# DaehwanKimLab/hisat-genotype

Measured on AMD Instinct MI355X. Metric: typed reads/sec at HLA-A (~7k alleles, 2x150bp), higher is better.
Workload: dtype u64 bitsets, f64 EM

## Files before the change

hisat-genotype_amd/capi.py:

```python
import ctypes as C
import threading
import os

import numpy as np

HERE = os.path.dirname(os.path.abspath(__file__))
LIB_PATH = os.path.join(HERE, "csrc", "libhgx.so")
LAB_PATH = os.path.join(HERE, "csrc", "lab", "libhgx_lab.so")

VAR_INSERTION, VAR_SINGLE, VAR_DELETION = 0, 1, 2
BASE_KIND = {"hla": 0, "codis": 1, "genome": 2}


class HgxError(RuntimeError):
    def __init__(self, code, msg):
        super().__init__("libhgx error %d: %s" % (code, msg))
        self.code = code


class HgxKeyError(HgxError, KeyError):
    """The reference raises KeyError at this point (EM quirk Q6)."""


class Piece(C.Structure):
    _fields_ = [("mask_off", C.c_uint32), ("lo_word", C.c_uint16), ("n_words", C.c_uint16)]


PIECE_DTYPE = np.dtype([("mask_off", np.uint32), ("lo_word", np.uint16), ("n_words", np.uint16)])


class LocusDesc(C.Structure):
    _fields_ = [("base_kind", C.c_int32), ("backbone_len", C.c_int32), ("backbone", C.c_char_p),
                ("n_vars", C.c_int32), ("var_pos", C.c_void_p), ("var_type", C.c_void_p), ("var_len", C.c_void_p),
                ("var_base", C.c_void_p), ("var_linked", C.c_void_p), ("var_name_pool", C.c_char_p),
                ("var_ins_pool", C.c_char_p), ("n_alleles", C.c_int32), ("link_off", C.c_void_p),
                ("link_allele", C.c_void_p), ("n_link_order", C.c_int32), ("link_order", C.c_void_p),
                ("n_exons", C.c_int32), ("exons", C.c_void_p), ("allele_len", C.c_void_p), ("name_rank", C.c_void_p)]


class ParseOpts(C.Structure):
    _fields_ = [("num_editdist", C.c_int32), ("error_correction", C.c_int32), ("allow_discordant", C.c_int32),
                ("simulation", C.c_int32), ("base_locus", C.c_int32), ("keep_trace", C.c_int32),
                ("codis_choose_pairs", C.c_int32), ("n_threads", C.c_int32),
                ("pileup_exchange", C.c_void_p), ("pileup_ctx", C.c_void_p),
                ("interdist_exchange", C.c_void_p), ("interdist_ctx", C.c_void_p),
                ("pileup_exchange_dev", C.c_void_p), ("pileup_dev_ctx", C.c_void_p)]


PILEUP_EXCHANGE = C.CFUNCTYPE(C.c_int, C.c_void_p, C.POINTER(C.c_uint32), C.c_int64)
PILEUP_EXCHANGE_DEV = C.CFUNCTYPE(C.c_int, C.c_void_p, C.c_void_p, C.c_int64, C.c_void_p)
INTERDIST_EXCHANGE = C.CFUNCTYPE(C.c_int, C.c_void_p, C.POINTER(C.c_int64), C.c_int64)


SYMBOLS = [
    "hgx_last_error", "hgx_version", "hgx_device_count", "hgx_set_device", "hgx_dev_alloc", "hgx_dev_free",
    "hgx_memcpy_h2d", "hgx_memcpy_h2d_async", "hgx_memcpy_d2h", "hgx_memset", "hgx_stream_sync", "hgx_stream_create", "hgx_stream_create_prio", "hgx_stream_destroy", "hgx_pool_trim", "hgx_event_create", "hgx_event_destroy",
    "hgx_event_record", "hgx_stream_wait_event", "hgx_event_elapsed_ms", "hgx_a_pad", "hgx_index_create",
    "hgx_index_destroy", "hgx_index_dims", "hgx_index_device_bits", "hgx_piece_compat", "hgx_pair_classes",
    "hgx_score_pairs", "hgx_level_classes", "hgx_group_pairs", "hgx_groups_dims", "hgx_groups_destroy",
    "hgx_level_classes_grouped", "hgx_classes_set_allele_rank", "hgx_dedup_classes", "hgx_classes_destroy", "hgx_classes_dims", "hgx_classes_device",
    "hgx_classes_to_host", "hgx_classes_from_host", "hgx_allele_counts", "hgx_allele_counts_on", "hgx_first_classes", "hgx_em", "hgx_em_ordered", "hgx_em_masked", "hgx_em_set_backend", "hgx_test_switch_set", "hgx_debug_matvec", "hgx_em_set_timing", "hgx_em_get_timing", "hgx_locus_create",
    "hgx_locus_destroy", "hgx_locus_dims", "hgx_locus_tables", "hgx_index_from_locus",
    "hgx_locus_alternatives_text", "hgx_batch_destroy", "hgx_batch_dims", "hgx_batch_arrays",
    "hgx_batch_from_haplotypes", "hgx_parse_sam", "hgx_read_alignments", "hgx_free_text", "hgx_parse_alignment_file", "hgx_batch_trace_text", "hgx_batch_pileup",
    "hgx_dbatch_create", "hgx_dbatch_destroy", "hgx_dbatch_dims", "hgx_gate_create", "hgx_gate_destroy", "hgx_type_dbatch",
    "hgx_type_batch", "hgx_type_file", "hgx_typing_destroy", "hgx_typing_dims", "hgx_typing_counts", "hgx_typing_em",
    "hgx_typing_gene_prob", "hgx_typing_classes", "hgx_write_bam", "hgx_em_last_exact", "hgx_index_device_block", "hgx_index_create_device", "hgx_type_classes", "hgx_pair_classes_dedup",
    "hgx_bgzf_inflate", "hgx_bgzf_inflate_verdicts", "hgx_bgzf_scan_compare", "hgx_many_create", "hgx_many_create_files", "hgx_many_create_sams", "hgx_many_tasks", "hgx_many_destroy", "hgx_many_dims", "hgx_type_many", "hgx_type_many_loci", "hgx_em_set_fast", "hgx_em_last_order", "hgx_typing_top", "hgx_emx_set_timing", "hgx_emx_get_timing",
    "hgx_index_broadcast", "hgx_allreduce_sum_u32", "hgx_allreduce_sum_i64", "hgx_classes_allgather",
    "hgx_classes_pack_rows", "hgx_classes_merge_gathered", "hgx_rccl_stats",
    "hgx_keyset_create", "hgx_keyset_dims", "hgx_keyset_fill", "hgx_keyset_destroy",
    "hgx_many_from_dbatch", "hgx_alignment_open", "hgx_alignment_dims", "hgx_alignment_parse_dev", "hgx_alignment_close", "hgx_stream_sets_info", "hgx_stream_create_placed", "hgx_stream_probe_matrix", "hgx_stream_probe_pair", "hgx_stream_probe_chain", "hgx_stream_sets_streams",
    "hgx_parse_sam_dev", "hgx_parse_alignment_file_dev", "hgx_front_last", "hgx_front_last_parts", "hgx_dbatch_to_host",
    "hgx_emx_cluster_stats", "hgx_em_tie_reruns",
    "hgx_linear_locus_create", "hgx_linear_locus_destroy", "hgx_linear_type_sam", "hgx_linear_type_file", "hgx_linear_dims",
    "hgx_linear_counts", "hgx_linear_classes", "hgx_linear_extra_names", "hgx_linear_destroy",
    "hgx_linear_input_open", "hgx_linear_input_dims", "hgx_linear_type_input", "hgx_linear_input_close",
    "hgx_alignment_set_open", "hgx_alignment_set_dims", "hgx_alignment_set_info", "hgx_alignment_set_route", "hgx_alignment_set_routed",
    "hgx_alignment_set_close", "hgx_many_create_set",
    "hgx_bam_index_build", "hgx_bam_index_last", "hgx_bam_splice",
    "hgx_extract_open", "hgx_extract_feed", "hgx_extract_feed_bam", "hgx_extract_file", "hgx_extract_take", "hgx_extract_stats", "hgx_extract_close",
    "hgx_align_index_create", "hgx_align_index_free", "hgx_align_reads", "hgx_align_last", "hgx_align_last_states",
    "hgx_align_last_pairs", "hgx_align_last_clip", "hgx_align_reads_x", "hgx_align_last_gap",
]

_lib = None


def lib():
    global _lib
    if _lib is None:
        if not os.path.exists(LIB_PATH):
            raise ImportError("libhgx.so is not built: run `python -c 'import __graft_entry__ as g; g.build()'` "
                              "(hipcc --offload-arch=gfx950); there is no CPU fallback")
        _lib = C.CDLL(LIB_PATH)
        _lib.hgx_last_error.restype = C.c_char_p
        _lib.hgx_a_pad.restype = C.c_int32
    return _lib


def use_lab():
    global LIB_PATH
    if _lib is not None:
        raise RuntimeError("libhgx.so is already loaded in this process")
    LIB_PATH = LAB_PATH


def check(rc):
    if rc != 0:
        msg = lib().hgx_last_error().decode(errors="replace")
        if rc == -4:
            raise HgxKeyError(rc, msg)
        raise HgxError(rc, msg)


def ptr(a):
    if a is None:
        return None
    if hasattr(a, "ptr") and not hasattr(a, "ctypes"):
        return C.c_void_p(a.ptr)
    return a.ctypes.data_as(C.c_void_p)


def a_pad(n_alleles):
    return int(lib().hgx_a_pad(C.c_int32(n_alleles)))


def device_count():
    n = C.c_int(0)
    check(lib().hgx_device_count(C.byref(n)))
    return n.value


_current_device = 0
_streams = {}


def set_device(dev):
    global _current_device
    check(lib().hgx_set_device(C.c_int(dev)))
    _current_device = dev


def current_device():
    return _current_device


_slot = threading.local()


def set_stream_slot(k):
    _slot.k = ("slot", k)


def get_stream(i):
    key = (_current_device, getattr(_slot, "k", threading.get_ident()), i)
    if key not in _streams:
        p = C.c_void_p()
        fn = lib().hgx_stream_create_placed if i == 2 else lib().hgx_stream_create_prio
        check(fn(C.byref(p), C.c_int(1 if i == 0 else 0)))
        _streams[key] = p
    return _streams[key]


class DevArray:

    def __init__(self, shape, dtype):
        self.shape = tuple(int(x) for x in (shape if isinstance(shape, (tuple, list)) else (shape,)))
        self.dtype = np.dtype(dtype)
        self.nbytes = int(np.prod(self.shape, dtype=np.int64)) * self.dtype.itemsize
        p = C.c_void_p()
        check(lib().hgx_dev_alloc(C.byref(p), C.c_size_t(self.nbytes)))
        self.ptr = p.value

    @staticmethod
    def from_host(arr, stream=None, sync=True):
        arr = np.ascontiguousarray(arr)
        d = DevArray(arr.shape, arr.dtype)
        if arr.nbytes:
            fn = lib().hgx_memcpy_h2d if sync else lib().hgx_memcpy_h2d_async
            check(fn(C.c_void_p(d.ptr), ptr(arr), C.c_size_t(arr.nbytes), stream))
        return d

    def to_host(self, stream=None):
        out = np.empty(self.shape, dtype=self.dtype)
        if self.nbytes:
            check(lib().hgx_memcpy_d2h(ptr(out), C.c_void_p(self.ptr), C.c_size_t(self.nbytes), stream))
        return out

    def zero(self, stream=None):
        check(lib().hgx_memset(C.c_void_p(self.ptr), 0, C.c_size_t(self.nbytes), stream))

    def free(self):
        if self.ptr:
            lib().hgx_dev_free(C.c_void_p(self.ptr))
            self.ptr = None

    def __del__(self):
        try:
            self.free()
        except Exception:
            pass


def sync(stream=None):
    check(lib().hgx_stream_sync(stream))


class Event:

    def __init__(self):
# ... 21 lines not shown
```

hisat-genotype_amd/csrc/hgx_device.hip:

```cpp
#include <hip/hip_runtime.h>

#include <algorithm>
#include <cstdarg>
#include <cstdio>
#include <cstring>
#include <vector>

#include <map>
#include <mutex>
#include <unordered_map>

#include "hgx_common.hpp"

static thread_local char g_err[512] = "";

extern "C" void hgx_set_error(const char *fmt, ...) {
    va_list ap;
    va_start(ap, fmt);
    vsnprintf(g_err, sizeof(g_err), fmt, ap);
    va_end(ap);
}
extern "C" const char *hgx_last_error(void) { return g_err; }
extern "C" int hgx_version(void) { return 100; }


extern "C" int hgx_device_count(int *n) { HIPCHK(hipGetDeviceCount(n)); return HGX_OK; }
namespace {
struct Staging {
    char *buf = nullptr;
    size_t cap = 0, used = 0;
    struct Pending { void *dst; const char *src; size_t n; };
    std::vector<Pending> pending;
    std::vector<hipStream_t> streams;
    void note(hipStream_t st) {
        for (auto s : streams) if (s == st) return;
        streams.push_back(st);
    }
    static std::mutex &mu() { static std::mutex m; return m; }
    static std::vector<char *> &free_list() { static std::vector<char *> v; return v; }
    ~Staging() {
        if (buf) { std::lock_guard<std::mutex> g(mu()); free_list().push_back(buf); }
    }
    char *take(size_t n) {
        const size_t need = (n + 63) & ~(size_t)63;
        if (!buf) {
            cap = 1u << 20;
            {
                std::lock_guard<std::mutex> g(mu());
                if (!free_list().empty()) { buf = free_list().back(); free_list().pop_back(); }
            }
            if (!buf && hipHostMalloc((void **)&buf, cap) != hipSuccess) { buf = nullptr; cap = 0; return nullptr; }
        }
        if (used + need > cap) return nullptr;
        char *r = buf + used;
        used += need;
        return r;
    }
};
thread_local Staging g_stage;
constexpr size_t STAGE_MAX = 256u << 10;
}

int hgx_d2h(void *dst, const void *src, size_t n, hipStream_t st) {
    char *s = n <= STAGE_MAX ? g_stage.take(n) : nullptr;
    if (!s) { HIPCHK(hipMemcpyAsync(dst, src, n, hipMemcpyDeviceToHost, st)); return HGX_OK; }
    HIPCHK(hipMemcpyAsync(s, src, n, hipMemcpyDeviceToHost, st));
    g_stage.pending.push_back({dst, s, n});
    g_stage.note(st);
    return HGX_OK;
}
int hgx_h2d(void *dst, const void *src, size_t n, hipStream_t st) {
    char *s = n <= STAGE_MAX ? g_stage.take(n) : nullptr;
    if (!s) { HIPCHK(hipMemcpyAsync(dst, src, n, hipMemcpyHostToDevice, st)); return HGX_OK; }
    memcpy(s, src, n);
    HIPCHK(hipMemcpyAsync(dst, s, n, hipMemcpyHostToDevice, st));
    g_stage.note(st);
    return HGX_OK;
}
int hgx_sync(hipStream_t st) {
    HIPCHK(hipStreamSynchronize(st));
    for (auto s2 : g_stage.streams) if (s2 != st) HIPCHK(hipStreamSynchronize(s2));
    g_stage.streams.clear();
    for (auto &p : g_stage.pending) memcpy(p.dst, p.src, p.n);
    g_stage.pending.clear();
    g_stage.used = 0;
    return HGX_OK;
}

extern "C" int hgx_set_device(int dev) { HIPCHK(hipSetDevice(dev)); return HGX_OK; }
void *hgx_pool_alloc(size_t bytes);
void hgx_pool_free(void *p);
extern "C" int hgx_dev_alloc(void **p, size_t bytes) {
    ARGCHK(p != nullptr);
    if (bytes <= (16u << 20)) {
        *p = hgx_pool_alloc(bytes);
        if (!*p) { hgx_set_error("device allocation of %zu bytes failed", bytes); return HGX_ENOMEM; }
        return HGX_OK;
    }
    HIPCHK(hipMalloc(p, bytes));
    return HGX_OK;
}
extern "C" int hgx_dev_free(void *p) { hgx_pool_free(p); return HGX_OK; }
extern "C" int hgx_memcpy_h2d(void *d, const void *s, size_t n, void *st) {
    int rc = hgx_h2d(d, s, n, (hipStream_t)st);
    return rc ? rc : hgx_sync((hipStream_t)st);
}
extern "C" int hgx_memcpy_h2d_async(void *d, const void *s, size_t n, void *st) {
    if (n > STAGE_MAX) return hgx_memcpy_h2d(d, s, n, st);
    return hgx_h2d(d, s, n, (hipStream_t)st);
}
extern "C" int hgx_memcpy_d2h(void *d, const void *s, size_t n, void *st) {
    int rc = hgx_d2h(d, s, n, (hipStream_t)st);
    return rc ? rc : hgx_sync((hipStream_t)st);
}
extern "C" int hgx_memset(void *d, int v, size_t n, void *st) {
    HIPCHK(hipMemsetAsync(d, v, n, (hipStream_t)st));
    return HGX_OK;
}
extern "C" int hgx_stream_sync(void *st) { return hgx_sync((hipStream_t)st); }
extern "C" int hgx_stream_create(void **st) {
    ARGCHK(st != nullptr);
    hipStream_t s;
    HIPCHK(hipStreamCreateWithFlags(&s, hipStreamNonBlocking));
    *st = (void *)s;
    return HGX_OK;
}
extern "C" int hgx_stream_create_prio(void **st, int high_priority) {
    ARGCHK(st != nullptr);
    int least = 0, greatest = 0;
    HIPCHK(hipDeviceGetStreamPriorityRange(&least, &greatest));
    hipStream_t s;
    HIPCHK(hipStreamCreateWithPriority(&s, hipStreamNonBlocking, high_priority ? greatest : least));
    *st = (void *)s;
    return HGX_OK;
}
bool hgx_ss_forget_stream(void *stream);
extern "C" int hgx_stream_destroy(void *st) {
    if (st && !hgx_ss_forget_stream(st)) HIPCHK(hipStreamDestroy((hipStream_t)st));
    return HGX_OK;
}
extern "C" int hgx_event_create(void **ev) {
    ARGCHK(ev != nullptr);
    hipEvent_t e;
    HIPCHK(hipEventCreate(&e));
    *ev = (void *)e;
    return HGX_OK;
}
extern "C" int hgx_event_destroy(void *ev) { if (ev) HIPCHK(hipEventDestroy((hipEvent_t)ev)); return HGX_OK; }
extern "C" int hgx_event_record(void *ev, void *st) { HIPCHK(hipEventRecord((hipEvent_t)ev, (hipStream_t)st)); return HGX_OK; }
extern "C" int hgx_stream_wait_event(void *st, void *ev) { HIPCHK(hipStreamWaitEvent((hipStream_t)st, (hipEvent_t)ev, 0)); return HGX_OK; }
extern "C" int hgx_event_elapsed_ms(void *a, void *b, float *ms) {
    ARGCHK(a && b && ms);
    HIPCHK(hipEventSynchronize((hipEvent_t)b));
    HIPCHK(hipEventElapsedTime(ms, (hipEvent_t)a, (hipEvent_t)b));
    return HGX_OK;
}


namespace {
struct Pool {
    std::mutex mu;
    std::multimap<std::pair<int, size_t>, void *> free_blocks;
    std::unordered_map<void *, std::pair<int, size_t>> size_of;
};
int cur_device() { int d = 0; (void)hipGetDevice(&d); return d; }
Pool &pool() { static Pool p; return p; }
size_t round_size(size_t n) {
    size_t r = 256;
    while (r < n) r <<= 1;
    if (r > (1u << 20)) {
        const size_t step = r >> 4;
        r = (n + step - 1) / step * step;
    }
    return r;
}
}

void *hgx_pool_alloc(size_t bytes) {
    Pool &P = pool();
    const size_t sz = round_size(bytes ? bytes : 8);
    const int dev = cur_device();
    {
        std::lock_guard<std::mutex> g(P.mu);
        auto it = P.free_blocks.find({dev, sz});
        if (it != P.free_blocks.end()) {
            void *p = it->second;
            P.free_blocks.erase(it);
            return p;
        }
    }
    void *p = nullptr;
    if (hipMalloc(&p, sz) != hipSuccess) {
        {
            std::lock_guard<std::mutex> g(P.mu);
            for (auto it = P.free_blocks.begin(); it != P.free_blocks.end();) {
                if (it->first.first == dev) { P.size_of.erase(it->second); (void)hipFree(it->second); it = P.free_blocks.erase(it); }
                else ++it;
            }
        }
        if (hipMalloc(&p, sz) != hipSuccess) return nullptr;
    }
    std::lock_guard<std::mutex> g(P.mu);
    P.size_of[p] = {dev, sz};
    return p;
}
void hgx_pool_free(void *p) {
    if (!p) return;
    Pool &P = pool();
    std::lock_guard<std::mutex> g(P.mu);
    auto it = P.size_of.find(p);
    if (it == P.size_of.end()) { (void)hipFree(p); return; }
    P.free_blocks.emplace(it->second, p);
}
void hgx_host_pool_trim();
extern "C" int hgx_pool_trim(void) {
    hgx_host_pool_trim();
    Pool &P = pool();
    std::lock_guard<std::mutex> g(P.mu);
    for (auto &kv : P.free_blocks) { P.size_of.erase(kv.second); (void)hipFree(kv.second); }
    P.free_blocks.clear();
    return HGX_OK;
}


extern "C" int32_t hgx_a_pad(int32_t n) { return (n + 511) / 512 * 512; }

static int index_alloc(hgx_index **out, int32_t n_alleles, int32_t n_vars) {
    ARGCHK(out && n_alleles > 0 && n_vars >= 0);
    ARGCHK(n_vars <= 65535 * 32);
    hgx_index *ix = new hgx_index();
    ix->n_alleles = n_alleles;
    ix->a_pad = hgx_a_pad(n_alleles);
    ix->n_vars = n_vars;
    ix->n_words = std::max(1, (n_vars + 31) / 32);
    ix->w64 = ix->a_pad / 64;
    const size_t nb = (size_t)ix->n_words * ix->a_pad * sizeof(uint32_t);
    void *block = nullptr;
    if (hipMalloc(&block, nb + 2 * (size_t)ix->w64 * 8) != hipSuccess) {
        delete ix;
        hgx_set_error("device allocation of the locus index failed");
        return HGX_ENOMEM;
    }
    ix->d_bits = (uint32_t *)block;
    ix->d_exon_mask = (uint64_t *)((char *)block + nb);
    ix->d_gene_mask = ix->d_exon_mask + ix->w64;
    *out = ix;
    return HGX_OK;
}
extern "C" int hgx_index_create(hgx_index **out, int32_t n_alleles, int32_t n_vars, const uint32_t *bits,
                                const uint64_t *exon_mask, const uint64_t *gene_mask) {
    ARGCHK(out && bits && exon_mask && gene_mask);
    *out = nullptr;
    hgx_index *ix = nullptr;
    { int rc_ = index_alloc(&ix, n_alleles, n_vars); if (rc_) return rc_; }
    const size_t nb = (size_t)ix->n_words * ix->a_pad * sizeof(uint32_t);
    if (hipMemcpy(ix->d_bits, bits, nb, hipMemcpyHostToDevice) != hipSuccess ||
        hipMemcpy(ix->d_exon_mask, exon_mask, ix->w64 * 8, hipMemcpyHostToDevice) != hipSuccess ||
        hipMemcpy(ix->d_gene_mask, gene_mask, ix->w64 * 8, hipMemcpyHostToDevice) != hipSuccess) {
        (void)hipFree(ix->d_bits);
        delete ix;
        hgx_set_error("upload of the locus index failed");
        return HGX_EHIP;
    }
    *out = ix;
    return HGX_OK;
}
extern "C" int hgx_index_create_device(hgx_index **out, int32_t n_alleles, int32_t n_vars) {
    ARGCHK(out);
    *out = nullptr;
    return index_alloc(out, n_alleles, n_vars);
}
extern "C" int hgx_index_destroy(hgx_index *ix) {
    if (!ix) return HGX_OK;
    (void)hipFree(ix->d_bits);
    hgx_pool_free(ix->d_pid); hgx_pool_free(ix->d_vals); hgx_pool_free(ix->d_nval);
    delete ix->pat_mu;
    delete ix;
    return HGX_OK;
}
extern "C" int hgx_index_dims(const hgx_index *ix, int32_t *na, int32_t *ap, int32_t *nv, int32_t *nw) {
    ARGCHK(ix);
    if (na) *na = ix->n_alleles;
    if (ap) *ap = ix->a_pad;
    if (nv) *nv = ix->n_vars;
    if (nw) *nw = ix->n_words;
    return HGX_OK;
}
extern "C" int hgx_index_device_bits(const hgx_index *ix, void **p, size_t *bytes) {
    ARGCHK(ix && p && bytes);
    *p = ix->d_bits;
    *bytes = (size_t)ix->n_words * ix->a_pad * sizeof(uint32_t);
// ... 341 lines not shown
        for (int s = 0; s < kw; ++s) {
            const int w = lane + 64 * s;
            const bool live = w < w64;
            uint64_t plane[NP];
#pragma unroll
            for (int k = 0; k < NP; ++k) plane[k] = 0;
            for (int r = r0; r < r1; ++r) {
                const uint32_t ref = (uint32_t)__builtin_amdgcn_readfirstlane(refs[r]);
                if ((ref >> 31) != level) continue;
                uint64_t carry = live ? compat[(size_t)(ref & 0x7fffffffu) * w64 + w] : 0ull;
#pragma unroll
                for (int k = 0; k < NP; ++k) {
                    const uint64_t t = plane[k] & carry;
                    plane[k] ^= carry;
                    carry = t;
                }
            }
            uint64_t cand = live ? mask[w] : 0ull;
            if (pass == 0) {
                uint32_t v = 0;
#pragma unroll
                for (int k = NP - 1; k >= 0; --k) {
                    const uint64_t t = cand & plane[k];
                    if (__any(t != 0)) { cand = t; v |= 1u << k; }
                }
                gmax = max(gmax, v);
            } else {
#pragma unroll
                for (int k = 0; k < NP; ++k) cand &= ((gmax >> k) & 1u) ? plane[k] : ~plane[k];
                if (live) {
#ifdef HGX_LAB
                    if (fa) __hip_atomic_store((unsigned long long *)&out_row[w], (unsigned long long)cand, __ATOMIC_RELAXED, __HIP_MEMORY_SCOPE_AGENT);
                    else
#endif
                    if (out_row) out_row[w] = cand;
                    h += word_hash(cand, w);
                    nz = nz || cand != 0;
                }
            }
        }
#ifdef HGX_LAB
    if (fa) {
        h = wave_sum_u64(h);
        const uint64_t key = finish_hash(h, __any(nz));
        if (key == HGX_EMPTY_KEY) { if (lane == 0) fa->slot_of[pair] = 0xFFFFFFFFu; return; }
        asm volatile("s_waitcnt vmcnt(0)" ::: "memory");
        int won;
        const uint32_t slot = fused_find_slot(*fa, key, lane, won);
        if (lane == 0) fa->slot_of[pair] = slot;
        if (won) { if (lane == 0) __hip_atomic_store(&fa->rep[slot], (uint32_t)pair, __ATOMIC_RELAXED, __HIP_MEMORY_SCOPE_AGENT); return; }
        const uint32_t r = fused_wait_rep(*fa, slot, lane);
        bool diff = false;
        for (int w = lane; w < w64; w += 64)
            diff = diff || __hip_atomic_load((unsigned long long *)&fa->rows[(size_t)r * w64 + w], __ATOMIC_RELAXED, __HIP_MEMORY_SCOPE_AGENT) !=
                               __hip_atomic_load((unsigned long long *)&out_row[w], __ATOMIC_RELAXED, __HIP_MEMORY_SCOPE_AGENT);
        if (__any(diff) && lane == 0) atomicOr(fa->bad, 1);
        return;
    }
#endif
    if (out_hash) {
        h = wave_sum_u64(h);
        const bool any_nz = __any(nz);
        if (lane == 0) *out_hash = finish_hash(h, any_nz);
    }
}

template <int KW, bool SEL>
__global__ __launch_bounds__(256) void k_pair_classes(const uint64_t *__restrict__ compat, int w64,
                                                      const int32_t *__restrict__ pair_off, const uint32_t *__restrict__ refs,
                                                      const int64_t *__restrict__ sel,
                                                      int n_pairs, const uint64_t *__restrict__ exon_mask,
                                                      const uint64_t *__restrict__ gene_mask, uint64_t *__restrict__ exon_bits,
                                                      uint64_t *__restrict__ gene_bits, uint64_t *__restrict__ exon_hash,
                                                      uint64_t *__restrict__ gene_hash) {
    const int lane = threadIdx.x & 63;
    const long out = ((long)blockIdx.x * blockDim.x + threadIdx.x) >> 6;
    if (out >= n_pairs) return;
    const long pair = SEL ? (long)sel[out] : out;
    const int r0 = __builtin_amdgcn_readfirstlane(pair_off[pair]);
    const int r1 = __builtin_amdgcn_readfirstlane(pair_off[pair + 1]);
    const int n_refs = r1 - r0;
#define HGX_LEVELS(NP_)                                                                                                          \
    do {                                                                                                                         \
        if (exon_bits || exon_hash)                                                                                              \
            class_for_level<KW, NP_>(compat, w64, refs, r0, r1, 0u, exon_mask, exon_bits ? exon_bits + (size_t)out * w64 : nullptr, \
                                     exon_hash ? exon_hash + out : nullptr, lane);                                              \
        if (gene_bits || gene_hash)                                                                                              \
            class_for_level<KW, NP_>(compat, w64, refs, r0, r1, 1u, gene_mask, gene_bits ? gene_bits + (size_t)out * w64 : nullptr, \
                                     gene_hash ? gene_hash + out : nullptr, lane);                                              \
    } while (0)
    if (n_refs <= 3) HGX_LEVELS(2);
    else if (n_refs <= 15) HGX_LEVELS(4);
    else if (n_refs <= 255) HGX_LEVELS(8);
    else {
        if (exon_bits || exon_hash)
            class_for_level_wide(compat, w64, refs, r0, r1, 0u, exon_mask, exon_bits ? exon_bits + (size_t)out * w64 : nullptr,
                                 exon_hash ? exon_hash + out : nullptr, lane);
        if (gene_bits || gene_hash)
            class_for_level_wide(compat, w64, refs, r0, r1, 1u, gene_mask, gene_bits ? gene_bits + (size_t)out * w64 : nullptr,
                                 gene_hash ? gene_hash + out : nullptr, lane);
    }
#undef HGX_LEVELS
}

template <int KW, int NP, bool FUSE = false>
__device__ __forceinline__ void two_classes(const uint64_t *__restrict__ compat, int w64, uint32_t ref_a, uint32_t ref_b,
                                            uint64_t todo_a, uint64_t todo_b, const uint64_t *__restrict__ mask,
                                            uint64_t *__restrict__ row_a, uint64_t *__restrict__ row_b,
                                            uint64_t *__restrict__ hash_a, uint64_t *__restrict__ hash_b, bool has_b, int lane,
                                            const FusedArgs *fa = nullptr, long pair_a = 0, long pair_b = 0) {
    uint64_t pa[NP][KW], pb[NP][KW];
#pragma unroll
    for (int k = 0; k < NP; ++k)
#pragma unroll
        for (int s = 0; s < KW; ++s) { pa[k][s] = 0; pb[k][s] = 0; }
    auto load_row = [&](uint32_t myref, uint64_t todo, uint64_t (&x)[KW]) {
        const uint64_t *row = compat + (size_t)((uint32_t)__builtin_amdgcn_readlane((int)myref, __builtin_ctzll(todo)) & 0x7fffffffu) * w64;
#pragma unroll
        for (int s = 0; s < KW; ++s) x[s] = (lane + 64 * s < w64) ? row[lane + 64 * s] : 0ull;
    };
    auto ripple = [&](uint64_t (&plane)[NP][KW], const uint64_t (&x)[KW]) {
        uint64_t carry[KW];
#pragma unroll
        for (int s = 0; s < KW; ++s) carry[s] = x[s];
#pragma unroll
        for (int k = 0; k < NP; ++k)
#pragma unroll
            for (int s = 0; s < KW; ++s) {
                const uint64_t t = plane[k][s] & carry[s];
                plane[k][s] ^= carry[s];
                carry[s] = t;
            }
    };
    uint64_t ca[KW], cb[KW], na[KW], nb[KW];
#pragma unroll
    for (int s = 0; s < KW; ++s) { ca[s] = 0; cb[s] = 0; na[s] = 0; nb[s] = 0; }
    if (todo_a) load_row(ref_a, todo_a, ca);
    if (todo_b) load_row(ref_b, todo_b, cb);
    while (todo_a | todo_b) {
        const bool have_a = todo_a != 0, have_b = todo_b != 0;
        todo_a &= todo_a - 1;
        todo_b &= todo_b - 1;
        if (todo_a) load_row(ref_a, todo_a, na);
        if (todo_b) load_row(ref_b, todo_b, nb);
        if (have_a) ripple(pa, ca);
        if (have_b) ripple(pb, cb);
#pragma unroll
        for (int s = 0; s < KW; ++s) { ca[s] = na[s]; cb[s] = nb[s]; }
    }
    emit_class<KW, NP, FUSE>(pa, w64, mask, row_a, hash_a, lane, fa, pair_a);
    if (has_b) emit_class<KW, NP, FUSE>(pb, w64, mask, row_b, hash_b, lane, fa, pair_b);
}

template <int KW, bool SEL>
__global__ __launch_bounds__(256) void k_pair_classes_x2(const uint64_t *__restrict__ compat, int w64,
                                                         const int32_t *__restrict__ pair_off, const uint32_t *__restrict__ refs,
                                                         const int64_t *__restrict__ sel, int n_pairs, uint32_t level,
                                                         const uint64_t *__restrict__ mask, uint64_t *__restrict__ bits,
                                                         uint64_t *__restrict__ hash) {
    const int lane = threadIdx.x & 63;
    const long out_a = (((long)blockIdx.x * blockDim.x + threadIdx.x) >> 6) * 2, out_b = out_a + 1;
    if (out_a >= n_pairs) return;
    const bool has_b = out_b < n_pairs;
    const long pair_a = SEL ? (long)sel[out_a] : out_a;
    const long pair_b = has_b ? (SEL ? (long)sel[out_b] : out_b) : pair_a;
    const int r0a = __builtin_amdgcn_readfirstlane(pair_off[pair_a]), r1a = __builtin_amdgcn_readfirstlane(pair_off[pair_a + 1]);
    const int r0b = __builtin_amdgcn_readfirstlane(pair_off[pair_b]), r1b = __builtin_amdgcn_readfirstlane(pair_off[pair_b + 1]);
    const int n_a = r1a - r0a, n_b = has_b ? r1b - r0b : 0;
    uint64_t *row_a = bits ? bits + (size_t)out_a * w64 : nullptr, *row_b = bits ? bits + (size_t)out_b * w64 : nullptr;
    uint64_t *hash_a = hash ? hash + out_a : nullptr, *hash_b = hash ? hash + out_b : nullptr;
    if (max(n_a, n_b) > 15) {
        if (n_a > 255) class_for_level_wide(compat, w64, refs, r0a, r1a, level, mask, row_a, hash_a, lane);
        else class_for_level<KW, 8>(compat, w64, refs, r0a, r1a, level, mask, row_a, hash_a, lane);
        if (has_b) {
            if (n_b > 255) class_for_level_wide(compat, w64, refs, r0b, r1b, level, mask, row_b, hash_b, lane);
            else class_for_level<KW, 8>(compat, w64, refs, r0b, r1b, level, mask, row_b, hash_b, lane);
        }
        return;
    }
    const uint32_t ref_a = lane < n_a ? refs[r0a + lane] : 0u, ref_b = lane < n_b ? refs[r0b + lane] : 0u;
    const uint64_t todo_a = __ballot(lane < n_a && (ref_a >> 31) == level), todo_b = __ballot(lane < n_b && (ref_b >> 31) == level);
    const int n_max = max(n_a, n_b);
    if (n_max <= 3) two_classes<KW, 2>(compat, w64, ref_a, ref_b, todo_a, todo_b, mask, row_a, row_b, hash_a, hash_b, has_b, lane);
    else two_classes<KW, 4>(compat, w64, ref_a, ref_b, todo_a, todo_b, mask, row_a, row_b, hash_a, hash_b, has_b, lane);
}

#ifdef HGX_LAB
#include "lab/hgx_fused_kernel_lab.inc"
#endif

int hgx_pair_classes_sel(const hgx_index *ix, const uint64_t *compat, const int32_t *pair_off, const uint32_t *refs,
                         const int64_t *sel, int32_t n_pairs, uint64_t *eb, uint64_t *gb, uint64_t *eh,
                         uint64_t *gh, hipStream_t st) {
    ARGCHK(ix && n_pairs >= 0);
    if (n_pairs == 0) return HGX_OK;
    ARGCHK(compat && pair_off && refs);
    const long blocks = ((long)n_pairs + 3) / 4;
    const int kw = (ix->w64 + 63) / 64;
    const bool exon = eb || eh, gene = gb || gh;
    if (exon != gene && kw <= 8 && !HGX_LAB_SWITCH("pair_x1")) {
        const long blocks2 = ((long)n_pairs + 7) / 8;
        const uint32_t level = gene ? 1u : 0u;
        const uint64_t *mask = gene ? ix->d_gene_mask : ix->d_exon_mask;
        uint64_t *bits = gene ? gb : eb, *hash = gene ? gh : eh;
#define LAUNCH_X2(KW_)                                                                                                        \
    do {                                                                                                                      \
        if (sel)                                                                                                              \
            hipLaunchKernelGGL((k_pair_classes_x2<KW_, true>), dim3((unsigned)blocks2), dim3(256), 0, st, compat, ix->w64, pair_off, \
                               refs, sel, n_pairs, level, mask, bits, hash);                                                  \
        else                                                                                                                  \
            hipLaunchKernelGGL((k_pair_classes_x2<KW_, false>), dim3((unsigned)blocks2), dim3(256), 0, st, compat, ix->w64, pair_off, \
                               refs, sel, n_pairs, level, mask, bits, hash);                                                  \
    } while (0)
        if (kw <= 1) LAUNCH_X2(1);
        else if (kw <= 2) LAUNCH_X2(2);
        else if (kw <= 4) LAUNCH_X2(4);
        else LAUNCH_X2(8);
#undef LAUNCH_X2
        HIPCHK(hipGetLastError());
        return HGX_OK;
    }
#define LAUNCH_PC(KW_)                                                                                                        \
    do {                                                                                                                      \
        if (sel)                                                                                                              \
            hipLaunchKernelGGL((k_pair_classes<KW_, true>), dim3((unsigned)blocks), dim3(256), 0, st, compat, ix->w64, pair_off, \
                               refs, sel, n_pairs, ix->d_exon_mask, ix->d_gene_mask, eb, gb, eh, gh);                        \
        else                                                                                                                  \
            hipLaunchKernelGGL((k_pair_classes<KW_, false>), dim3((unsigned)blocks), dim3(256), 0, st, compat, ix->w64, pair_off, \
                               refs, sel, n_pairs, ix->d_exon_mask, ix->d_gene_mask, eb, gb, eh, gh);                        \
    } while (0)
    if (kw <= 1) LAUNCH_PC(1);
    else if (kw <= 2) LAUNCH_PC(2);
    else if (kw <= 4) LAUNCH_PC(4);
    else if (kw <= 8) LAUNCH_PC(8);
    else {
        hgx_set_error("more than 32768 alleles per locus are not supported (a_pad=%d)", ix->a_pad);
        return HGX_EINVAL;
    }
#undef LAUNCH_PC
    HIPCHK(hipGetLastError());
    return HGX_OK;
}

extern "C" int hgx_pair_classes(const hgx_index *ix, const uint64_t *compat, const int32_t *pair_off, const uint32_t *refs,
                                int32_t n_pairs, uint64_t *eb, uint64_t *gb, uint64_t *eh, uint64_t *gh, void *stream) {
    return hgx_pair_classes_sel(ix, compat, pair_off, refs, nullptr, n_pairs, eb, gb, eh, gh, (hipStream_t)stream);
}

extern "C" int hgx_score_pairs(const hgx_index *ix, const hgx_piece *pieces, const uint32_t *masks, int32_t n_pieces,
                               const int32_t *pair_off, const uint32_t *refs, int32_t n_pairs, uint64_t *compat,
                               uint64_t *eb, uint64_t *gb, uint64_t *eh, uint64_t *gh, void *stream) {
    int rc = hgx_piece_compat(ix, pieces, masks, n_pieces, compat, stream);
    if (rc) return rc;
    return hgx_pair_classes(ix, compat, pair_off, refs, n_pairs, eb, gb, eh, gh, stream);
}
```

include/hgx.h:

```cpp
#ifndef HGX_H
#define HGX_H

#include <stddef.h>
#include <stdint.h>

#ifdef __cplusplus
extern "C" {
#endif

#define HGX_OK            0
#define HGX_EINVAL       -1
#define HGX_EHIP         -2
#define HGX_ENOMEM       -3
#define HGX_EKEY         -4
#define HGX_ECOLLISION   -5
#define HGX_EPARSE       -6
#define HGX_ETYPE        -7

#define HGX_VAR_INSERTION 0
#define HGX_VAR_SINGLE    1
#define HGX_VAR_DELETION  2

#define HGX_LEVEL_EXON 0
#define HGX_LEVEL_GENE 1

const char *hgx_last_error(void);
int hgx_version(void);

int hgx_device_count(int *n);
int hgx_set_device(int dev);
int hgx_dev_alloc(void **dev_ptr, size_t bytes);
int hgx_dev_free(void *dev_ptr);
int hgx_memcpy_h2d(void *dev_dst, const void *host_src, size_t bytes, void *stream);
int hgx_memcpy_h2d_async(void *dst_dev, const void *src_host, size_t bytes, void *stream);
int hgx_memcpy_d2h(void *host_dst, const void *dev_src, size_t bytes, void *stream);
int hgx_memset(void *dev_dst, int value, size_t bytes, void *stream);
int hgx_stream_sync(void *stream);
int hgx_stream_create(void **stream);
int hgx_stream_create_prio(void **stream, int high_priority);
int hgx_stream_destroy(void *stream);
int hgx_pool_trim(void);
int hgx_event_create(void **event);
int hgx_event_destroy(void *event);
int hgx_event_record(void *event, void *stream);
int hgx_stream_wait_event(void *stream, void *event);
int hgx_event_elapsed_ms(void *start_event, void *stop_event, float *ms);

typedef struct hgx_index hgx_index;

int32_t hgx_a_pad(int32_t n_alleles);
int hgx_index_create(hgx_index **out,
                     int32_t n_alleles, int32_t n_vars,
                     const uint32_t *link_bits_host,
                     const uint64_t *exon_allele_mask,
                     const uint64_t *gene_allele_mask);
int hgx_index_destroy(hgx_index *ix);
int hgx_index_dims(const hgx_index *ix, int32_t *n_alleles, int32_t *a_pad, int32_t *n_vars, int32_t *n_words);
int hgx_index_device_bits(const hgx_index *ix, void **dev_bits, size_t *bytes);
int hgx_index_device_block(const hgx_index *ix, void **dev_block, size_t *bytes);
int hgx_index_create_device(hgx_index **out, int32_t n_alleles, int32_t n_vars);

int hgx_index_broadcast(hgx_index *ix, int32_t root, void *rccl_comm, void *stream);
int hgx_allreduce_sum_u32(uint32_t *dev_buf, size_t n, void *rccl_comm, void *stream);
int hgx_allreduce_sum_i64(int64_t *dev_buf, size_t n, void *rccl_comm, void *stream);

typedef struct hgx_piece {
    uint32_t mask_off;
    uint16_t lo_word;
    uint16_t n_words;
} hgx_piece;

int hgx_piece_compat(const hgx_index *ix, const hgx_piece *pieces_dev, const uint32_t *masks_dev,
                     int32_t n_pieces, uint64_t *compat_dev, void *stream);

int hgx_pair_classes(const hgx_index *ix, const uint64_t *compat_dev,
                     const int32_t *pair_off_dev,
                     const uint32_t *pair_ref_dev, int32_t n_pairs,
                     uint64_t *exon_bits_dev,
                     uint64_t *gene_bits_dev,
                     uint64_t *exon_hash_dev,
                     uint64_t *gene_hash_dev,
                     void *stream);

int hgx_score_pairs(const hgx_index *ix,
                    const hgx_piece *pieces_dev, const uint32_t *masks_dev, int32_t n_pieces,
                    const int32_t *pair_off_dev, const uint32_t *pair_ref_dev, int32_t n_pairs,
                    uint64_t *compat_scratch_dev,
                    uint64_t *exon_bits_dev, uint64_t *gene_bits_dev,
                    uint64_t *exon_hash_dev, uint64_t *gene_hash_dev,
                    void *stream);

typedef struct hgx_classes hgx_classes;

int hgx_dedup_classes(hgx_classes **out,
                      const uint64_t *rows_dev, const uint64_t *row_hash_dev_or_null,
                      const int64_t *row_weight_dev_or_null,
                      int64_t n_rows, int32_t a_pad,
                      const uint64_t *and_mask_dev_or_null,
                      void *stream);
int hgx_classes_destroy(hgx_classes *c);
int hgx_classes_dims(const hgx_classes *c, int32_t *n_classes, int32_t *a_pad);
int hgx_classes_device(const hgx_classes *c, void **bits_dev, void **count_dev ,
                       void **first_row_dev );
int hgx_classes_to_host(const hgx_classes *c, uint64_t *bits_host, int64_t *count_host, int64_t *first_row_host);
int hgx_classes_from_host(hgx_classes **out, const uint64_t *bits_host, const int64_t *count_host,
                          int32_t n_classes, int32_t a_pad);
int hgx_classes_allgather(hgx_classes **out, const hgx_classes *mine_or_null, int32_t a_pad, void *rccl_comm, void *stream);
int hgx_classes_pack_rows(const hgx_classes *mine_or_null, int32_t a_pad, int32_t cap, void *dev_send, void *stream);
int hgx_classes_merge_gathered(hgx_classes **out, const void *dev_recv, const int32_t *sizes_host, int32_t world, int32_t cap,
                               int32_t a_pad, void *stream);
int hgx_rccl_stats(uint64_t *n_collectives, uint64_t *bytes_sent, uint64_t *bytes_received, int32_t reset);

int hgx_level_classes(hgx_classes **out, const hgx_index *ix, const uint64_t *compat_dev,
                      const int32_t *pair_off_dev, const uint32_t *pair_ref_dev, int32_t n_pairs, int32_t level,
                      uint64_t *rows_scratch_dev, uint64_t *hash_scratch_dev, void *stream);
typedef struct hgx_groups hgx_groups;
int hgx_group_pairs(hgx_groups **out, const int32_t *pair_off_dev, const uint32_t *pair_ref_dev, int32_t n_pairs,
                    int32_t level, void *stream);
int hgx_groups_dims(hgx_groups *g, int64_t *n_groups, int32_t *n_pairs);
int hgx_groups_destroy(hgx_groups *g);
int hgx_level_classes_grouped(hgx_classes **out, const hgx_index *ix, const uint64_t *compat_dev,
                              const int32_t *pair_off_dev, const uint32_t *pair_ref_dev, hgx_groups *groups,
                              uint64_t *rows_scratch_dev, uint64_t *hash_scratch_dev, void *stream);

int hgx_pair_classes_dedup(hgx_classes **out, const hgx_index *ix, const uint64_t *compat_dev, const int32_t *pair_off_dev,
                           const uint32_t *pair_ref_dev, int32_t n_pairs, int32_t level, uint64_t *rows_scratch_dev, void *stream);

int hgx_allele_counts(const hgx_classes *c, int64_t *count_host, int32_t *first_class_host);
int hgx_allele_counts_on(const hgx_classes *c, int64_t *count_host, int32_t *first_class_host, void *stream);
int hgx_first_classes(const hgx_classes *c, const int32_t *alleles_host, int32_t n, int32_t *first_class_host, void *stream);

typedef struct hgx_keyset hgx_keyset;
int hgx_keyset_create(hgx_keyset **out, const char *keys, size_t n_bytes, int32_t n_keys);
int hgx_keyset_dims(const hgx_keyset *ks, int32_t *n_names, int32_t *a_pad, size_t *name_pool_bytes, int32_t *keys_sorted);
int hgx_keyset_fill(const hgx_keyset *ks, uint64_t *bits_host, char *name_pool, int32_t *name_rank);
int hgx_keyset_destroy(hgx_keyset *ks);

int hgx_em(const hgx_classes *c, int32_t n_alleles,
           int32_t remove_low, const int32_t *allele_len_or_null ,
           double *prob_host, int32_t *n_iter_host, void *stream);
int hgx_em_ordered(const hgx_classes *c, int32_t n_alleles, int32_t remove_low, const int32_t *allele_len_or_null,
                   double *prob_host, int32_t *first_class_host, int32_t *n_iter_host, void *stream);

int hgx_classes_set_allele_rank(hgx_classes *c, const int32_t *rank_host, int32_t n);
int hgx_em_last_exact(void);
int hgx_em_last_order(int32_t *order_host, int32_t n_alleles);
int hgx_em_set_fast(int on);

int hgx_em_masked(const hgx_classes *c, const uint64_t *mask_host, int32_t n_alleles, int32_t remove_low,
                  const int32_t *allele_len_or_null, double *prob_host, int32_t *first_class_host, int32_t *n_iter_host,
                  int32_t *n_classes_host, void *stream);

#define HGX_BASE_HLA    0
#define HGX_BASE_CODIS  1
#define HGX_BASE_GENOME 2
#define HGX_BASE_OTHER  3

typedef struct hgx_locus_desc {
    int32_t base_kind;
    int32_t backbone_len;
    const char *backbone;
    int32_t n_vars;
    const int32_t *var_pos;
    const uint8_t *var_type;
    const int32_t *var_len;
    const char *var_base;
    const uint8_t *var_linked;
    const char *var_name_pool;
    const char *var_ins_pool;
    int32_t n_alleles;
    const int32_t *link_off;
    const int32_t *link_allele;
    int32_t n_link_order;
    const int32_t *link_order;
    int32_t n_exons;
    const int32_t *exons;
    const int32_t *allele_len;
    const int32_t *name_rank;
} hgx_locus_desc;

typedef struct hgx_locus hgx_locus;
int hgx_locus_create(hgx_locus **out, const hgx_locus_desc *desc);
int hgx_locus_destroy(hgx_locus *loc);
int hgx_locus_dims(const hgx_locus *loc, int32_t *n_alleles, int32_t *a_pad, int32_t *n_vars, int32_t *n_words);
int hgx_locus_tables(const hgx_locus *loc, uint32_t *link_bits, uint64_t *exon_mask, uint64_t *gene_mask,
                     int32_t *rep_of);
int hgx_index_from_locus(hgx_index **out, const hgx_locus *loc);
int hgx_locus_alternatives_text(const hgx_locus *loc, char *buf, size_t cap, size_t *needed);

typedef struct hgx_batch hgx_batch;
int hgx_batch_destroy(hgx_batch *b);
int hgx_batch_dims(const hgx_batch *b, int32_t *n_pieces, int64_t *n_mask_u32, int32_t *n_pairs, int64_t *n_refs,
                   int32_t *n_reads);
int hgx_batch_arrays(const hgx_batch *b, const hgx_piece **pieces, const uint32_t **masks, const int32_t **pair_off,
                     const uint32_t **pair_ref);

int hgx_batch_from_haplotypes(hgx_batch **out, const hgx_locus *loc, int32_t n_pairs, const int32_t *pair_off,
                              const uint8_t *piece_level, const int32_t *piece_left, const int32_t *piece_right,
                              const int32_t *piece_id_off, const int32_t *piece_ids);

typedef struct hgx_parse_opts {
    int32_t num_editdist;
    int32_t error_correction;
    int32_t allow_discordant;
    int32_t simulation;
    int32_t base_locus;
    int32_t keep_trace;
    int32_t codis_choose_pairs;
    int32_t n_threads;
    int (*pileup_exchange)(void *ctx, uint32_t *counts, int64_t n_cells);
    void *pileup_ctx;
    int (*interdist_exchange)(void *ctx, int64_t *hist, int64_t n_bins);
    void *interdist_ctx;
    int (*pileup_exchange_dev)(void *ctx, uint32_t *d_counts, int64_t n, void *stream);
    void *pileup_dev_ctx;
} hgx_parse_opts;
#define HGX_INTERDIST_HALF 65536
#define HGX_INTERDIST_BINS (2 * HGX_INTERDIST_HALF + 2)

int hgx_parse_sam(hgx_batch **out, const hgx_locus *loc, const char *sam, size_t n_bytes, const hgx_parse_opts *opts);

#define HGX_MAX_REGIONS 8
int hgx_read_alignments(const char *path, const char *regions_or_null, int32_t n_threads, char **text_out, size_t *n_bytes_out);
int hgx_free_text(char *text);
int hgx_parse_alignment_file(hgx_batch **out, const hgx_locus *loc, const char *path, const char *regions_or_null,
                             const hgx_parse_opts *opts);
int hgx_write_bam(const char *path, const char *sam, size_t n_bytes, const char *ref_names, const int32_t *ref_lens, int32_t n_refs,
                  int32_t sort_by_coordinate, int32_t n_threads);
int hgx_batch_trace_text(const hgx_batch *b, char *buf, size_t cap, size_t *needed);
int hgx_batch_pileup(const hgx_batch *b, uint8_t *nt_set, uint32_t *counts);

typedef struct hgx_typing hgx_typing;
typedef struct hgx_dbatch hgx_dbatch;
typedef struct hgx_gate hgx_gate;
typedef struct hgx_type_opts {
// ... 171 lines not shown
```

Measured before the change: 487.6 million.

## Split pair-class kernel into hot/mid paths and defer rare wide pairs

The pair-class kernel now classifies each pair by how many references it has at the requested level. Pairs with three or fewer get a specialised two-plane bit-count path, and pairs with up to fifteen get a four-plane path. Pairs above that are appended through an atomic counter to a per-stream device list and handled by a second kernel, one wavefront per pair. The aim is to keep wavefronts in the main kernel free of the long serial loops that stalled whole wavefronts on rare wide pairs. In exchange it adds a second launch, a persistent per-stream scratch buffer, and self-resetting counters that assume one launch at a time per stream.

```diff
diff --git a/hisat-genotype_amd/capi.py b/hisat-genotype_amd/capi.py
--- a/hisat-genotype_amd/capi.py
+++ b/hisat-genotype_amd/capi.py
@@ -56,7 +56,7 @@
     "hgx_last_error", "hgx_version", "hgx_device_count", "hgx_set_device", "hgx_dev_alloc", "hgx_dev_free",
     "hgx_memcpy_h2d", "hgx_memcpy_h2d_async", "hgx_memcpy_d2h", "hgx_memset", "hgx_stream_sync", "hgx_stream_create", "hgx_stream_create_prio", "hgx_stream_destroy", "hgx_pool_trim", "hgx_event_create", "hgx_event_destroy",
     "hgx_event_record", "hgx_stream_wait_event", "hgx_event_elapsed_ms", "hgx_a_pad", "hgx_index_create",
-    "hgx_index_destroy", "hgx_index_dims", "hgx_index_device_bits", "hgx_piece_compat", "hgx_pair_classes",
+    "hgx_index_destroy", "hgx_index_dims", "hgx_index_device_bits", "hgx_piece_compat", "hgx_pair_classes", "hgx_pair_rest_wavefronts",
     "hgx_score_pairs", "hgx_level_classes", "hgx_group_pairs", "hgx_groups_dims", "hgx_groups_destroy",
     "hgx_level_classes_grouped", "hgx_classes_set_allele_rank", "hgx_dedup_classes", "hgx_classes_destroy", "hgx_classes_dims", "hgx_classes_device",
     "hgx_classes_to_host", "hgx_classes_from_host", "hgx_allele_counts", "hgx_allele_counts_on", "hgx_first_classes", "hgx_em", "hgx_em_ordered", "hgx_em_masked", "hgx_em_set_backend", "hgx_test_switch_set", "hgx_debug_matvec", "hgx_em_set_timing", "hgx_em_get_timing", "hgx_locus_create",
diff --git a/hisat-genotype_amd/csrc/hgx_device.hip b/hisat-genotype_amd/csrc/hgx_device.hip
--- a/hisat-genotype_amd/csrc/hgx_device.hip
+++ b/hisat-genotype_amd/csrc/hgx_device.hip
@@ -135,8 +135,12 @@
     return HGX_OK;
 }
 bool hgx_ss_forget_stream(void *stream);
+void hgx_pair_list_forget(hipStream_t st);
 extern "C" int hgx_stream_destroy(void *st) {
-    if (st && !hgx_ss_forget_stream(st)) HIPCHK(hipStreamDestroy((hipStream_t)st));
+    if (st && !hgx_ss_forget_stream(st)) {
+        hgx_pair_list_forget((hipStream_t)st);
+        HIPCHK(hipStreamDestroy((hipStream_t)st));
+    }
     return HGX_OK;
 }
 extern "C" int hgx_event_create(void **ev) {
@@ -784,12 +788,85 @@
     if (has_b) emit_class<KW, NP, FUSE>(pb, w64, mask, row_b, hash_b, lane, fa, pair_b);
 }
 
+constexpr int PAIR_HOT_REFS = 3;
+constexpr int PAIR_MID_REFS = 15;
+constexpr int PAIR_REST_HEAD = 2;
+constexpr int PAIR_REST_THREADS = 64;
+constexpr int PAIR_REST_BLOCKS = 512;
+
+template <int KW>
+__device__ __forceinline__ void hot_rows(const uint64_t *__restrict__ compat, int w64, uint32_t myref, uint64_t todo,
+                                         uint64_t (&x)[PAIR_HOT_REFS][KW], int lane) {
+#pragma unroll
+    for (int i = 0; i < PAIR_HOT_REFS; ++i) {
+#pragma unroll
+        for (int s = 0; s < KW; ++s) x[i][s] = 0;
+        if (todo) {
+            const uint64_t *row = compat + (size_t)((uint32_t)__builtin_amdgcn_readlane((int)myref, __builtin_ctzll(todo)) & 0x7fffffffu) * w64;
+#pragma unroll
+            for (int s = 0; s < KW; ++s)
+                if (lane + 64 * s < w64) x[i][s] = row[lane + 64 * s];
+        }
+        todo &= todo - 1;
+    }
+}
+template <int KW>
+__device__ __forceinline__ void hot_class(const uint64_t (&x)[PAIR_HOT_REFS][KW], int w64, const uint64_t *__restrict__ mask,
+                                          uint64_t *__restrict__ out_row, uint64_t *__restrict__ out_hash, int lane) {
+    static_assert(PAIR_HOT_REFS == 3, "two planes hold the counts of three rows");
+    uint64_t plane[2][KW];
+#pragma unroll
+    for (int s = 0; s < KW; ++s) {
+        const uint64_t t = x[0][s] ^ x[1][s];
+        plane[0][s] = t ^ x[2][s];
+        plane[1][s] = (x[0][s] & x[1][s]) | (t & x[2][s]);
+    }
+    emit_class<KW, 2>(plane, w64, mask, out_row, out_hash, lane);
+}
+
+template <int KW>
+__device__ __forceinline__ void mid_class(const uint64_t *__restrict__ compat, int w64, uint32_t myref, uint64_t todo,
+                                          const uint64_t *__restrict__ mask, uint64_t *__restrict__ out_row,
+                                          uint64_t *__restrict__ out_hash, int lane) {
+    constexpr int NP = 4;
+    static_assert(PAIR_MID_REFS < (1 << NP), "four planes hold the counts");
+    uint64_t plane[NP][KW], cur[KW], nxt[KW];
+#pragma unroll
+    for (int k = 0; k < NP; ++k)
+#pragma unroll
+        for (int s = 0; s < KW; ++s) plane[k][s] = 0;
+    auto load_row = [&](uint64_t t, uint64_t (&x)[KW]) {
+        const uint64_t *row = compat + (size_t)((uint32_t)__builtin_amdgcn_readlane((int)myref, __builtin_ctzll(t)) & 0x7fffffffu) * w64;
+#pragma unroll
+        for (int s = 0; s < KW; ++s) x[s] = (lane + 64 * s < w64) ? row[lane + 64 * s] : 0ull;
+    };
+#pragma unroll
+    for (int s = 0; s < KW; ++s) { cur[s] = 0; nxt[s] = 0; }
+    if (todo) load_row(todo, cur);
+    while (todo) {
+        todo &= todo - 1;
+        if (todo) load_row(todo, nxt);
+#pragma unroll
+        for (int s = 0; s < KW; ++s) {
+            uint64_t carry = cur[s];
+#pragma unroll
+            for (int k = 0; k < NP; ++k) {
+                const uint64_t t = plane[k][s] & carry;
+                plane[k][s] ^= carry;
+                carry = t;
+            }
+            cur[s] = nxt[s];
+        }
+    }
+    emit_class<KW, NP>(plane, w64, mask, out_row, out_hash, lane);
+}
+
 template <int KW, bool SEL>
 __global__ __launch_bounds__(256) void k_pair_classes_x2(const uint64_t *__restrict__ compat, int w64,
                                                          const int32_t *__restrict__ pair_off, const uint32_t *__restrict__ refs,
                                                          const int64_t *__restrict__ sel, int n_pairs, uint32_t level,
                                                          const uint64_t *__restrict__ mask, uint64_t *__restrict__ bits,
-                                                         uint64_t *__restrict__ hash) {
+                                                         uint64_t *__restrict__ hash, uint32_t *__restrict__ rest) {
     const int lane = threadIdx.x & 63;
     const long out_a = (((long)blockIdx.x * blockDim.x + threadIdx.x) >> 6) * 2, out_b = out_a + 1;
     if (out_a >= n_pairs) return;
@@ -799,27 +876,97 @@
     const int r0a = __builtin_amdgcn_readfirstlane(pair_off[pair_a]), r1a = __builtin_amdgcn_readfirstlane(pair_off[pair_a + 1]);
     const int r0b = __builtin_amdgcn_readfirstlane(pair_off[pair_b]), r1b = __builtin_amdgcn_readfirstlane(pair_off[pair_b + 1]);
     const int n_a = r1a - r0a, n_b = has_b ? r1b - r0b : 0;
+    const bool fit_a = n_a <= 64, fit_b = n_b <= 64;
+    const uint32_t ref_a = (fit_a && lane < n_a) ? refs[r0a + lane] : 0u, ref_b = (fit_b && lane < n_b) ? refs[r0b + lane] : 0u;
+    uint64_t todo_a = __ballot(fit_a && lane < n_a && (ref_a >> 31) == level);
+    uint64_t todo_b = __ballot(fit_b && lane < n_b && (ref_b >> 31) == level);
+    const int c_a = fit_a ? __popcll(todo_a) : PAIR_MID_REFS + 1, c_b = !has_b ? 0 : fit_b ? __popcll(todo_b) : PAIR_MID_REFS + 1;
+    const bool rare_a = c_a > PAIR_MID_REFS, rare_b = c_b > PAIR_MID_REFS;
+    if (rare_a || rare_b) {
+        if (lane == 0) {
+            uint32_t at = atomicAdd(&rest[0], (uint32_t)rare_a + (uint32_t)rare_b);
+            if (rare_a) rest[PAIR_REST_HEAD + at++] = (uint32_t)out_a;
+            if (rare_b) rest[PAIR_REST_HEAD + at] = (uint32_t)out_b;
+        }
+    }
     uint64_t *row_a = bits ? bits + (size_t)out_a * w64 : nullptr, *row_b = bits ? bits + (size_t)out_b * w64 : nullptr;
     uint64_t *hash_a = hash ? hash + out_a : nullptr, *hash_b = hash ? hash + out_b : nullptr;
-    if (max(n_a, n_b) > 15) {
-        if (n_a > 255) class_for_level_wide(compat, w64, refs, r0a, r1a, level, mask, row_a, hash_a, lane);
-        else class_for_level<KW, 8>(compat, w64, refs, r0a, r1a, level, mask, row_a, hash_a, lane);
-        if (has_b) {
-            if (n_b > 255) class_for_level_wide(compat, w64, refs, r0b, r1b, level, mask, row_b, hash_b, lane);
-            else class_for_level<KW, 8>(compat, w64, refs, r0b, r1b, level, mask, row_b, hash_b, lane);
-        }
-        return;
-    }
-    const uint32_t ref_a = lane < n_a ? refs[r0a + lane] : 0u, ref_b = lane < n_b ? refs[r0b + lane] : 0u;
-    const uint64_t todo_a = __ballot(lane < n_a && (ref_a >> 31) == level), todo_b = __ballot(lane < n_b && (ref_b >> 31) == level);
-    const int n_max = max(n_a, n_b);
-    if (n_max <= 3) two_classes<KW, 2>(compat, w64, ref_a, ref_b, todo_a, todo_b, mask, row_a, row_b, hash_a, hash_b, has_b, lane);
-    else two_classes<KW, 4>(compat, w64, ref_a, ref_b, todo_a, todo_b, mask, row_a, row_b, hash_a, hash_b, has_b, lane);
+    const bool hot_a = c_a <= PAIR_HOT_REFS, hot_b = has_b && c_b <= PAIR_HOT_REFS;
+    {
+        uint64_t xa[PAIR_HOT_REFS][KW], xb[PAIR_HOT_REFS][KW];
+        hot_rows<KW>(compat, w64, ref_a, hot_a ? todo_a : 0ull, xa, lane);
+        hot_rows<KW>(compat, w64, ref_b, hot_b ? todo_b : 0ull, xb, lane);
+        if (hot_a) hot_class<KW>(xa, w64, mask, row_a, hash_a, lane);
+        if (hot_b) hot_class<KW>(xb, w64, mask, row_b, hash_b, lane);
+    }
+    if (!hot_a && !rare_a) mid_class<KW>(compat, w64, ref_a, todo_a, mask, row_a, hash_a, lane);
+    if (!hot_b && !rare_b && has_b) mid_class<KW>(compat, w64, ref_b, todo_b, mask, row_b, hash_b, lane);
+}
+
+template <int KW, bool SEL>
+__global__ __launch_bounds__(PAIR_REST_THREADS) void k_pair_classes_rest(const uint64_t *__restrict__ compat, int w64,
+                                                           const int32_t *__restrict__ pair_off, const uint32_t *__restrict__ refs,
+                                                           const int64_t *__restrict__ sel, uint32_t level,
+                                                           const uint64_t *__restrict__ mask, uint64_t *__restrict__ bits,
+                                                           uint64_t *__restrict__ hash, uint32_t *rest) {
+    const int lane = threadIdx.x & 63;
+    const uint32_t n_list = (uint32_t)__builtin_amdgcn_readfirstlane((int)__hip_atomic_load(&rest[0], __ATOMIC_RELAXED, __HIP_MEMORY_SCOPE_AGENT));
+    __syncthreads();
+    if (threadIdx.x == 0 && atomicAdd(&rest[1], 1u) == gridDim.x - 1) {
+        __hip_atomic_store(&rest[0], 0u, __ATOMIC_RELAXED, __HIP_MEMORY_SCOPE_AGENT);
+        __hip_atomic_store(&rest[1], 0u, __ATOMIC_RELAXED, __HIP_MEMORY_SCOPE_AGENT);
+    }
+    for (uint32_t i = blockIdx.x * (PAIR_REST_THREADS / 64) + (threadIdx.x >> 6); i < n_list; i += gridDim.x * (PAIR_REST_THREADS / 64)) {
+        const long out = (long)(uint32_t)__builtin_amdgcn_readfirstlane((int)rest[PAIR_REST_HEAD + i]);
+        const long pair = SEL ? (long)sel[out] : out;
+        const int r0 = __builtin_amdgcn_readfirstlane(pair_off[pair]), r1 = __builtin_amdgcn_readfirstlane(pair_off[pair + 1]);
+        int n_lv = 0;
+        for (int base = r0; base < r1; base += 64) {
+            const int r = base + lane;
+            n_lv += __popcll(__ballot(r < r1 && (refs[r < r1 ? r : r0] >> 31) == level));
+        }
+        uint64_t *row = bits ? bits + (size_t)out * w64 : nullptr, *h = hash ? hash + out : nullptr;
+        if (n_lv <= 15) class_for_level<KW, 4>(compat, w64, refs, r0, r1, level, mask, row, h, lane);
+        else if (n_lv <= 255) class_for_level<KW, 8>(compat, w64, refs, r0, r1, level, mask, row, h, lane);
+        else class_for_level_wide(compat, w64, refs, r0, r1, level, mask, row, h, lane);
+    }
 }
 
 #ifdef HGX_LAB
 #include "lab/hgx_fused_kernel_lab.inc"
 #endif
+
+namespace {
+struct PairList { uint32_t *p = nullptr; size_t cap = 0; };
+std::mutex g_pair_list_mu;
+std::map<std::pair<int, hipStream_t>, PairList> g_pair_list;
+}
+static int pair_list_get(hipStream_t st, size_t n_entries, uint32_t **out) {
+    std::lock_guard<std::mutex> g(g_pair_list_mu);
+    PairList &pl = g_pair_list[{cur_device(), st}];
+    if (pl.cap < n_entries) {
+        if (pl.p) { HIPCHK(hipStreamSynchronize(st)); hgx_pool_free(pl.p); pl.p = nullptr; pl.cap = 0; }
+        const size_t cap = std::max<size_t>(n_entries, 1024);
+        uint32_t *p = (uint32_t *)hgx_pool_alloc((PAIR_REST_HEAD + cap) * 4);
+        if (!p) { hgx_set_error("device allocation of %zu bytes failed", (PAIR_REST_HEAD + cap) * 4); return HGX_ENOMEM; }
+        if (hipMemsetAsync(p, 0, PAIR_REST_HEAD * 4, st) != hipSuccess) { hgx_pool_free(p); hgx_set_error("hipMemsetAsync failed"); return HGX_EHIP; }
+        pl.p = p;
+        pl.cap = cap;
+    }
+    *out = pl.p;
+    return HGX_OK;
+}
+void hgx_pair_list_forget(hipStream_t st) {
+    std::lock_guard<std::mutex> g(g_pair_list_mu);
+    for (auto it = g_pair_list.begin(); it != g_pair_list.end();) {
+        if (it->first.second == st) {
+            (void)hipStreamSynchronize(st);
+            hgx_pool_free(it->second.p);
+            it = g_pair_list.erase(it);
+        } else ++it;
+    }
+}
+extern "C" int32_t hgx_pair_rest_wavefronts(void) { return PAIR_REST_BLOCKS * (PAIR_REST_THREADS / 64); }
 
 int hgx_pair_classes_sel(const hgx_index *ix, const uint64_t *compat, const int32_t *pair_off, const uint32_t *refs,
                          const int64_t *sel, int32_t n_pairs, uint64_t *eb, uint64_t *gb, uint64_t *eh,
@@ -835,14 +982,22 @@
         const uint32_t level = gene ? 1u : 0u;
         const uint64_t *mask = gene ? ix->d_gene_mask : ix->d_exon_mask;
         uint64_t *bits = gene ? gb : eb, *hash = gene ? gh : eh;
+        uint32_t *rest = nullptr;
+        TRY(pair_list_get(st, (size_t)n_pairs, &rest));
+        const unsigned rest_blocks = (unsigned)std::min<long>(PAIR_REST_BLOCKS, n_pairs);
 #define LAUNCH_X2(KW_)                                                                                                        \
     do {                                                                                                                      \
-        if (sel)                                                                                                              \
+        if (sel) {                                                                                                            \
             hipLaunchKernelGGL((k_pair_classes_x2<KW_, true>), dim3((unsigned)blocks2), dim3(256), 0, st, compat, ix->w64, pair_off, \
-                               refs, sel, n_pairs, level, mask, bits, hash);                                                  \
-        else                                                                                                                  \
+                               refs, sel, n_pairs, level, mask, bits, hash, rest);                                            \
+            hipLaunchKernelGGL((k_pair_classes_rest<KW_, true>), dim3(rest_blocks), dim3(PAIR_REST_THREADS), 0, st, compat, ix->w64, \
+                               pair_off, refs, sel, level, mask, bits, hash, rest);                                           \
+        } else {                                                                                                              \
             hipLaunchKernelGGL((k_pair_classes_x2<KW_, false>), dim3((unsigned)blocks2), dim3(256), 0, st, compat, ix->w64, pair_off, \
-                               refs, sel, n_pairs, level, mask, bits, hash);                                                  \
+                               refs, sel, n_pairs, level, mask, bits, hash, rest);                                            \
+            hipLaunchKernelGGL((k_pair_classes_rest<KW_, false>), dim3(rest_blocks), dim3(PAIR_REST_THREADS), 0, st, compat, ix->w64, \
+                               pair_off, refs, sel, level, mask, bits, hash, rest);                                           \
+        }                                                                                                                     \
     } while (0)
         if (kw <= 1) LAUNCH_X2(1);
         else if (kw <= 2) LAUNCH_X2(2);
diff --git a/include/hgx.h b/include/hgx.h
--- a/include/hgx.h
+++ b/include/hgx.h
@@ -81,6 +81,7 @@
                      uint64_t *exon_hash_dev,
                      uint64_t *gene_hash_dev,
                      void *stream);
+int32_t hgx_pair_rest_wavefronts(void);
 
 int hgx_score_pairs(const hgx_index *ix,
                     const hgx_piece *pieces_dev, const uint32_t *masks_dev, int32_t n_pieces,
```

Result: slower. 482.5 million (-1.0%).
